# ErikNatanael/knaster

Hardware: AMD Instinct MI355X
Metric: UGen-samples/sec (voices x block_size x UGens / s) (higher is better)
Workload: dtype f32

## Files before the change

knaster_amd/csrc/voice_chain.hpp:

```cpp
#pragma once
#include "voice_stages.hpp"

namespace knh_dev {

template <typename F, bool FMA, int BASE, typename... S> struct Chain;
template <typename F, bool FMA, int BASE>
struct Chain<F, FMA, BASE> {
  static constexpr int kSlots = BASE;
  static constexpr bool kUsesSine = false;
  static constexpr bool kPan = false;
  static constexpr bool kStereo = false;
  static constexpr u64 kParamBits = 0ull, kNopOkBits = 0ull;
  static constexpr bool kBinds = false;
  static constexpr bool kUsesRing = false;
  static constexpr int kRingStages = 0;
  template <int T> __device__ __forceinline__ void tick_tile_sw(const Chain&, u32, u64, F (&)[T], const Ctx&, u32) {}
  __device__ __forceinline__ void pan_gains(F&, F&) const {}
  template <typename W> __device__ __forceinline__ void load(const W*, long) {}
  template <typename W> __device__ __forceinline__ void store(W*, long) const {}
  __device__ __forceinline__ F tick(F x, const Ctx&, u32) { return x; }
  template <int T> __device__ __forceinline__ void tick_tile(F (&)[T], const Ctx&, u32) {}
  struct RunPrep {};
  __device__ __forceinline__ RunPrep prepare_run() const { return RunPrep(); }
  template <int T> __device__ __forceinline__ void tick_tile_run(F (&)[T], const Ctx&, u32, const RunPrep&) {}
#ifdef KNH_DAG_STAMPS
  template <int T> __device__ __forceinline__ void tick_tile_stamped(F (&)[T], const Ctx&, u32, u64*, u64&) {}
#endif
  __device__ __forceinline__ void on_event(u32, u32, u64, u32) {}
  __device__ __forceinline__ bool last_env_stopped(bool dflt) const { return dflt; }
  __device__ __forceinline__ u32 collect_done(u32 acc) const { return acc; }
  __device__ __forceinline__ void reset_marks() {}
  __device__ __forceinline__ void begin_block(u32, const Ctx&) {}
};
template <typename F, bool FMA, int BASE, typename S0, typename... Rest>
struct Chain<F, FMA, BASE, S0, Rest...> {
  typedef Chain<F, FMA, BASE + S0::kSlots, Rest...> RestT;
  static constexpr int kSlots = RestT::kSlots;
  static constexpr bool kUsesSine = S0::kUsesSine || RestT::kUsesSine;
  static constexpr bool kPan = IsPan<S0>::value || RestT::kPan;
  static constexpr bool kStereo = false;
  static constexpr u64 kStageBits = BASE + S0::kSlots <= 64 ? (((u64)1 << S0::kSlots) - 1) << (BASE < 64 ? BASE : 0) : 0ull;
  static constexpr u64 kParamBits = (BASE + S0::kSlots <= 64 ? (u64)S0::kParamMask << (BASE < 64 ? BASE : 0) : 0ull) | RestT::kParamBits;
  static constexpr u64 kNopOkBits = ((S0::kParamMask != 0u || !S0::kHasSeg) && BASE < 64 ? (u64)1 << (BASE < 64 ? BASE : 0) : 0ull) | RestT::kNopOkBits;
  static constexpr bool kBinds = S0::kNeedsBind || RestT::kBinds;
  static constexpr bool kUsesRing = S0::kUsesRing || RestT::kUsesRing;
  static constexpr int kRingStages = (S0::kUsesRing ? 1 : 0) + RestT::kRingStages;
  typename S0::template Regs<F> r;
  u32 mark = 0xFFFFFFFFu;
  RestT rest;
  template <typename W> __device__ __forceinline__ void load(const W* s, long stride) {
    S0::template load<F, W>(r, s + (long)BASE * stride, stride);
    rest.load(s, stride);
  }
  template <typename W> __device__ __forceinline__ void store(W* s, long stride) const {
    S0::template store<F, W>(r, s + (long)BASE * stride, stride);
    rest.store(s, stride);
  }
  __device__ __forceinline__ F tick(F x, const Ctx& c, u32 frame) {
    x = S0::template tick<F, FMA>(r, x, c, frame, mark);
    return rest.tick(x, c, frame);
  }
  template <int T> __device__ __forceinline__ void tick_tile(F (&x)[T], const Ctx& c, u32 frame0) {
    S0::template tick_tile<F, FMA, T>(r, x, c, frame0, mark);
    rest.template tick_tile<T>(x, c, frame0);
  }
  struct RunPrep { bool mine; typename RestT::RunPrep rest; };
  __device__ __forceinline__ RunPrep prepare_run() const {
    RunPrep p;
    if constexpr (S0::kHasRunPrep) p.mine = S0::template prepare_run<F>(r);
    else p.mine = false;
    p.rest = rest.prepare_run();
    return p;
  }
  template <int T> __device__ __forceinline__ void tick_tile_run(F (&x)[T], const Ctx& c, u32 frame0, const RunPrep& p) {
    if constexpr (S0::kHasRunPrep) S0::template tick_tile_prepared<F, FMA, T>(r, x, c, frame0, mark, p.mine);
    else S0::template tick_tile<F, FMA, T>(r, x, c, frame0, mark);
    rest.template tick_tile_run<T>(x, c, frame0, p.rest);
  }
#ifdef KNH_DAG_STAMPS
  template <int T> __device__ __forceinline__ void tick_tile_stamped(F (&x)[T], const Ctx& c, u32 frame0, u64* acc, u64& t_prev) {
    S0::template tick_tile<F, FMA, T>(r, x, c, frame0, mark);
    asm volatile("" : "+v"(x[T - 1]) : : "memory");
    const u64 t = __builtin_amdgcn_s_memtime();
    acc[0] += t - t_prev;
    t_prev = t;
    rest.template tick_tile_stamped<T>(x, c, frame0, acc + 1, t_prev);
  }
#endif
  template <int T> __device__ __forceinline__ void tick_tile_sw(const Chain& cn, u32 sw, u64 touched, F (&x)[T], const Ctx& c, u32 frame0) {
    bool hit = false;
    if constexpr (S0::kParamMask != 0u) hit = __builtin_amdgcn_ballot_w64((touched & kStageBits) != 0ull) != 0;
    if (hit) {
#pragma unroll
      for (int j = 0; j < T; ++j) {
        S0::take_params(r, cn.r, (u32)j == sw);
        x[j] = S0::template tick<F, FMA>(r, x[j], c, frame0 + j, mark);
      }
    } else {
#pragma unroll
      for (int j = 0; j < T; ++j) x[j] = S0::template tick<F, FMA>(r, x[j], c, frame0 + j, mark);
    }
    rest.template tick_tile_sw<T>(cn.rest, sw, touched, x, c, frame0);
  }
  __device__ __forceinline__ u32 collect_done(u32 acc) const {
    if constexpr (S0::kIsEnv) acc = mark != 0xFFFFFFFFu ? mark : acc;
    return rest.collect_done(acc);
  }
  __device__ __forceinline__ void reset_marks() { mark = 0xFFFFFFFFu; rest.reset_marks(); }
  __device__ __forceinline__ void pan_gains(F& l, F& rg) const {
    if constexpr (IsPan<S0>::value) { l = r.l; rg = r.r; }
    else rest.pan_gains(l, rg);
  }
  __device__ __forceinline__ void on_event(u32 op, u32 slot, u64 bits, u32 frame) {
    if (slot >= (u32)BASE && slot < (u32)(BASE + S0::kSlots)) S0::template on_event<F>(r, op, slot - BASE, bits, frame);
    else rest.on_event(op, slot, bits, frame);
  }
  __device__ __forceinline__ bool last_env_stopped(bool dflt) const {
    if constexpr (S0::kIsEnv && !S0::kEnvSource) return rest.last_env_stopped(S0::template is_stopped<F>(r));
    else return rest.last_env_stopped(dflt);
  }
  __device__ __forceinline__ void begin_block(u32 frame_begin, const Ctx& c) {
    if constexpr (S0::kNeedsBind) S0::template bind<F>(r, c);
    if constexpr (S0::kIsEnv && S0::kHasSeg) r.seg = frame_begin;
    rest.begin_block(frame_begin, c);
  }
};

template <int OP>
struct Math2 : StageDefaults {
  static constexpr int kSlots = 0;
  static constexpr u32 kMutableMask = 0u;
  static constexpr bool kUsesSine = false;
  static constexpr bool kIsEnv = false;
  static constexpr bool kNeedsBind = false;
  static constexpr bool kHasSeg = false;
  static constexpr bool kBinary = true;
  template <typename F> struct Regs {};
  template <typename F, typename W> static __device__ __forceinline__ void load(Regs<F>&, const W*, long) {}
  template <typename F, typename W> static __device__ __forceinline__ void store(const Regs<F>&, W*, long) {}
  template <typename F> static __device__ __forceinline__ F apply(F a, F b) {
    if (OP == 0) return a * b;
    if (OP == 1) return a + b;
    if (OP == 2) return a - b;
    if (OP == 3) return a / b;
    return dev_pow(a, b);
  }
  template <typename F, bool FMA> static __device__ __forceinline__ F tick(Regs<F>&, F x, const Ctx&, u32, u32&) { return x; }
  template <typename F, bool FMA, int T> static __device__ __forceinline__ void tick_tile(Regs<F>&, F (&)[T], const Ctx&, u32, u32&) {}
  template <typename F> static __device__ __forceinline__ void on_event(Regs<F>&, u32, u32, u64, u32) {}
};
template <typename S, int A, int B, int O> struct At {};
template <typename S, int A, int B, int O, int O2> struct At2 {};
template <int R> struct Slots {};
template <int R, int K> struct Out1 {};
template <int R, int L, int RR> struct Outs {};
template <typename X> struct NodeOf { static constexpr bool dag = false; };
template <typename S, int A, int B, int O> struct NodeOf<At<S, A, B, O>> { typedef S stage; static constexpr int a = A, b = B, o = O, o2 = -1; static constexpr bool dag = true; };
template <typename S, int A, int B, int O, int O2> struct NodeOf<At2<S, A, B, O, O2>> { typedef S stage; static constexpr int a = A, b = B, o = O, o2 = O2; static constexpr bool dag = true; };
template <int R> struct NodeOf<Slots<R>> { static constexpr bool dag = true; };
template <int R, int K> struct NodeOf<Out1<R, K>> { static constexpr bool dag = true; };
template <int R, int L, int RR> struct NodeOf<Outs<R, L, RR>> { static constexpr bool dag = true; };

template <typename F, bool FMA, int BASE, int R, int LAST, typename... Ns> struct DagChain;
template <typename F, int BASE, int R>
struct DagEnd {
  static constexpr int kSlots = BASE;
  static constexpr bool kUsesSine = false;
  static constexpr bool kPan = false;
  static constexpr bool kUsesRing = false;
  static constexpr int kRingStages = 0;
  __device__ __forceinline__ void pan_gains(F&, F&) const {}
  template <typename W> __device__ __forceinline__ void load(const W*, long) {}
  template <typename W> __device__ __forceinline__ void store(W*, long) const {}
  template <int T> __device__ __forceinline__ void run_tile(F (&)[R][T], const Ctx&, u32) {}
  __device__ __forceinline__ void run_one(F (&)[R], const Ctx&, u32) {}
  __device__ __forceinline__ void on_event(u32, u32, u64, u32) {}
  __device__ __forceinline__ bool last_env_stopped(bool dflt) const { return dflt; }
// ... 1046 lines not shown
```

knaster_amd/csrc/voice_pipe.hpp:

```cpp
#pragma once
#include "voice_chain.hpp"

namespace knh_dev {

template <typename... S> struct Group {};
template <int K, typename... S> struct Fan {};

template <typename G> struct GroupInfo;
template <typename... S> struct GroupInfo<Group<S...>> {
  static constexpr int slots = (0 + ... + S::kSlots);
  static constexpr bool uses_sine = (false || ... || S::kUsesSine);
  static constexpr bool uses_ring = (false || ... || S::kUsesRing);
  static constexpr bool has_env = (false || ... || S::kIsEnv);
  static constexpr bool has_silencer = (false || ... || (S::kIsEnv && !S::kEnvSource));
  static constexpr bool pan = (false || ... || IsPan<S>::value);
  static constexpr int fan_for(int) { return 1; }
};
template <int K, typename... S> struct GroupInfo<Fan<K, S...>> {
  static constexpr int slots = (0 + ... + S::kSlots);
  static constexpr bool uses_sine = (false || ... || S::kUsesSine);
  static constexpr bool uses_ring = false;
  static constexpr bool has_env = false;
  static constexpr bool has_silencer = false;
  static constexpr bool pan = false;
// ... 135 lines not shown
    if (ev_i < ev_end) { nxt = fetch(ev_ranged ? 2u * ev_i : ev_i); note_next(); }
    else { nxt.frame = 0xFFFFFFFFu; next_frame = 0xFFFFFFFFu; }
  };
  u32 base = 0;
  auto apply_events_upto = [&](u32 n_abs) {
    while (__builtin_expect(next_frame <= n_abs, 0)) {
      const u32 op = nxt.slot_op >> 24, slot = nxt.slot_op & 0xFFFFFFu;
      if (slot >= SLOT_LO && slot < SLOT_HI) {
        chain.on_event(op, slot, nxt.bits, nxt.frame - base);
        if (live && (op & 0x7Fu) == EV_SET) a.state[(long)slot * a.stride + voice] = (W)nxt.bits;
      }
      ++ev_i;
      take_next();
    }
  };
  u32 done_frame = 0xFFFFFFFFu;
  for (;;) {
  if (resident) {
    const ResCall call = res_wait(a.res, res_expect, sh.res_slot, wave_all, lane);
    if (call.leave) break;
    res_expect = (res_expect + 1u) & (u32)RES_EPOCH_MASK;
    fbeg = call.frame_begin;
    fend = call.frame_end;
    evs = call.has_events ? a.res.ev_start[call.list] : nullptr;
    ev_g = (glb_ev_t)a.res.events[call.list];
    chain.reset_marks();
    const ResStaged st = res_stage_events(a.res, call, sh.ev_stage, sh.ev_cap, v0, nv, (u32)(wave_all * 64 + lane), sh.n_threads);
    ev_staged = st.count != 0u;
    ev_lds_first = st.first;
    ev_ranged = call.has_events && call.n_ranges != 0u;
    if (ev_ranged) { evs = nullptr; ev_i = 0; ev_end = call.n_ranges; }
  } else if (sh.launch_ranges != 0u) {
    ev_ranged = true;
    ev_i = 0; ev_end = sh.launch_ranges;
  }
  if (!ev_ranged) {
    ev_i = 0; ev_end = 0;
    if (evs) {
      if (resident) { ev_i = *reinterpret_cast<const volatile u32*>(evs + voice); ev_end = *reinterpret_cast<const volatile u32*>(evs + voice + 1); }
      else { ev_i = evs[voice]; ev_end = evs[voice + 1]; }
    }
  }
  nxt.frame = 0xFFFFFFFFu; next_frame = 0xFFFFFFFFu;
  take_next();
  base = 0;

  const u32 n_frames = fend - fbeg;
  const int tpb = (int)((n_frames + T - 1) / T);
  const int n_tiles = tpb * (int)a.n_blocks;
  const int n_steps = n_tiles + NG - (MODE == PIPE_FOLD ? 1 : 0);
  const u32 n_waves_total = (a.n_voices + 63u) / 64u;
  const int full = n_frames >= fo + (u32)TW ? (int)((n_frames - fo - (u32)TW) / (u32)T) + 1 : 0;
  int in_t = Map::in_tile(I, 0), out_t = Map::out_tile(I, 0);
#ifdef KNH_DAG_STAMPS
  u64 busy = 0, busy_in = 0, busy_out = 0, busy_tick = 0, busy_fold = 0;
#endif
  for (int s = 0; s < I; ++s) pipe_barrier();
  for (int blk = 0, ti = 0; blk < (tpb > 0 ? (int)a.n_blocks : 0); ++blk) {
    ctx.input_block = reinterpret_cast<const F*>(a.input) + (long)blk * a.in_channels * a.block_size;
    chain.begin_block(fbeg, ctx);
    for (ti = 0;;) {
      typedef typename EdgeLayout<F, T>::Vec Vec;
      constexpr int VW = EdgeLayout<F, T>::VW;
#ifdef KNH_DAG_STAMPS
      const u64 t0 = __builtin_amdgcn_s_memtime();
#endif
      const u32 n_tile = fbeg + (u32)ti * T;
      const u32 n = n_tile + fo;
      apply_events_upto(base + n);
      const bool ev_inside = next_frame < base + n + TW;
      bool step_open = true;
      if (__builtin_expect(ti < full && !__builtin_amdgcn_ballot_w64(ev_inside), 1)) {
        const typename ChainT::RunPrep prep = chain.prepare_run();
        u32 nq = n;
        for (;;) {
#ifdef KNH_DAG_STAMPS
          const u64 q0 = __builtin_amdgcn_s_memtime();
#endif
          F x[TW];
          if (I > 0) {
            const Vec* in = reinterpret_cast<const Vec*>(sh.edge + (long)in_t * EdgeLayout<F, T>::tile + (long)lane * EdgeLayout<F, T>::stride + fo);
#pragma unroll
            for (int j = 0; j < TW / VW; ++j) {
              const Vec v = in[j];
#pragma unroll
              for (int k = 0; k < VW; ++k) x[j * VW + k] = v[k];
            }
          } else {
#pragma unroll
            for (int j = 0; j < TW; ++j) x[j] = (F)0;
          }
#if defined(KNH_DAG_STAMPS) || defined(KNH_TILE_FENCES)
          asm volatile("s_waitcnt lgkmcnt(0)" ::: "memory");
#endif
#ifdef KNH_DAG_STAMPS
          const u64 q1 = __builtin_amdgcn_s_memtime();
          busy_in += q1 - q0;
#endif
          chain.template tick_tile_run<TW>(x, ctx, nq, prep);
#ifdef KNH_DAG_STAMPS
          asm volatile("" ::: "memory");
          const u64 q2 = __builtin_amdgcn_s_memtime();
          busy_tick += q2 - q1;
#endif
          F* const out_tile = sh.edge + (long)out_t * EdgeLayout<F, T>::tile;
          F* const out_row = out_tile + (long)lane * EdgeLayout<F, T>::stride + fo;
          Vec* out = reinterpret_cast<Vec*>(out_row);
#pragma unroll
          for (int j = 0; j < TW / VW; ++j) {
            Vec v;
#pragma unroll
            for (int k = 0; k < VW; ++k) v[k] = x[j * VW + k];
            out[j] = v;
          }
          if constexpr (GroupInfo<G>::pan) {
            F gl = (F)0, gr = (F)0;
            chain.pan_gains(gl, gr);
            out_row[T] = gl;
            out_row[T + 1] = gr;
          }
#ifdef KNH_DAG_STAMPS
          asm volatile("s_waitcnt lgkmcnt(0)" ::: "memory");
          const u64 qf = __builtin_amdgcn_s_memtime();
#endif
          if constexpr (FOLDS) pipe_fold_tile<F, FMA, T, GroupInfo<G>::pan>(out_tile, a, lane, wave_global, n_waves_total, blk, nq, (u32)T, v0, nv);
#ifdef KNH_DAG_STAMPS
          asm volatile("s_waitcnt lgkmcnt(0)" ::: "memory");
          const u64 qe = __builtin_amdgcn_s_memtime();
          busy_fold += qe - qf;
#endif
          in_t = Map::next_in(I, in_t);
          out_t = Map::next_out(I, out_t);
          nq += (u32)T;
          ++ti;
#if defined(KNH_DAG_STAMPS) || defined(KNH_TILE_FENCES)
          asm volatile("s_waitcnt lgkmcnt(0)" ::: "memory");
#endif
#ifdef KNH_DAG_STAMPS
          const u64 q3 = __builtin_amdgcn_s_memtime();
          busy_out += q3 - qe;
          busy += q3 - q0;
#endif
          if (ti >= full) break;
          pipe_barrier();
          if (__builtin_amdgcn_ballot_w64(next_frame < base + nq + TW)) { step_open = false; break; }
        }
      } else {
        const u32 m_tile = fend - n_tile < (u32)T ? fend - n_tile : (u32)T;
        const u32 m = m_tile > fo ? (m_tile - fo < (u32)TW ? m_tile - fo : (u32)TW) : 0u;
        F* const out_tile = sh.edge + (long)out_t * EdgeLayout<F, T>::tile;
        F* const out_row = out_tile + (long)lane * EdgeLayout<F, T>::stride + fo;
        const F* const in_row = sh.edge + (long)in_t * EdgeLayout<F, T>::tile + (long)lane * EdgeLayout<F, T>::stride + fo;
#ifdef KNH_AB_NO_SW
        if (false && [&]() -> bool {
#else
        if (m == (u32)TW && ChainT::kParamBits != 0ull && !ChainT::kBinds && [&]() -> bool {
#endif
          ChainT cn = chain;
          const u32 sv_i = ev_i;
          const Event sv_nxt = nxt;
          const u32 sv_next_frame = next_frame;
          const u32 tile_end = base + n + (u32)TW;
          u32 sw = (u32)TW;
          u64 touched = 0ull;
          bool bad = false;
          while (next_frame < tile_end) {
            const u32 op = nxt.slot_op >> 24, slot = nxt.slot_op & 0xFFFFFFu, code = op & 0x7Fu;
            if (slot >= SLOT_LO && slot < SLOT_HI) {
              const u32 rel = nxt.frame - (base + n);
              if (sw == (u32)TW) sw = rel;
              bad = bad || sw != rel || slot >= 64u ||
                    !((code == EV_SET && ((ChainT::kParamBits >> (slot & 63u)) & 1ull)) || (code == EV_NOP && ((ChainT::kNopOkBits >> (slot & 63u)) & 1ull)));
              if (!bad) {
                cn.on_event(op, slot, nxt.bits, nxt.frame - base);
                touched |= 1ull << (slot & 63u);
                if (live && code == EV_SET) a.state[(long)slot * a.stride + voice] = (W)nxt.bits;
              }
            }
            ++ev_i;
            take_next();
          }
          if (__builtin_amdgcn_ballot_w64(bad) != 0) {
            ev_i = sv_i;
            nxt = sv_nxt;
            next_frame = sv_next_frame;
            return false;
          }
          for (u32 j0 = 0; j0 < (u32)TW; j0 += 8u) {
            F sub[8];
            if (I > 0) {
#pragma unroll
              for (int q = 0; q < 8 / VW; ++q) {
                const Vec v = reinterpret_cast<const Vec*>(in_row + j0)[q];
#pragma unroll
                for (int k = 0; k < VW; ++k) sub[q * VW + k] = v[k];
              }
            } else {
#pragma unroll
// ... 348 lines not shown
```

knaster_amd/csrc/voice_stages.hpp:

```cpp
#pragma once

extern "C" __device__ float __ocml_sin_f32(float);
extern "C" __device__ double __ocml_sin_f64(double);
extern "C" __device__ float __ocml_cos_f32(float);
extern "C" __device__ double __ocml_cos_f64(double);
extern "C" __device__ float __ocml_pow_f32(float, float);
extern "C" __device__ double __ocml_pow_f64(double, double);
extern "C" __device__ float __ocml_tan_f32(float);
extern "C" __device__ double __ocml_tan_f64(double);
extern "C" __device__ float __ocml_exp_f32(float);
extern "C" __device__ double __ocml_exp_f64(double);
extern "C" __device__ float __ocml_sqrt_f32(float);
extern "C" __device__ double __ocml_sqrt_f64(double);

namespace knh_dev {

typedef unsigned int u32;
typedef unsigned long long u64;

template <typename F> struct WordOf;
template <> struct WordOf<float> { typedef u32 type; };
template <> struct WordOf<double> { typedef u64 type; };

template <typename F> __device__ __forceinline__ F word_to_f(typename WordOf<F>::type w);
template <> __device__ __forceinline__ float word_to_f<float>(u32 w) { return __builtin_bit_cast(float, w); }
template <> __device__ __forceinline__ double word_to_f<double>(u64 w) { return __builtin_bit_cast(double, w); }
__device__ __forceinline__ u32 f_to_word(float f) { return __builtin_bit_cast(u32, f); }
__device__ __forceinline__ u64 f_to_word(double f) { return __builtin_bit_cast(u64, f); }

template <bool FMA> __device__ __forceinline__ float mad(float a, float b, float c) {
  if constexpr (FMA) return __builtin_fmaf(a, b, c);
  else return a * b + c;
}
template <bool FMA> __device__ __forceinline__ double mad(double a, double b, double c) {
  if constexpr (FMA) return __builtin_fma(a, b, c);
  else return a * b + c;
}

__device__ __forceinline__ u32 sat_u32(double v) {
  u32 r;
  asm("v_cvt_u32_f64 %0, %1" : "=v"(r) : "v"(v));
  return r;
}

struct StageDefaults {
  static constexpr u32 kParamMask = 0u;
  template <typename R> static __device__ __forceinline__ void take_params(R&, const R&, bool) {}
  static constexpr bool kBinary = false;
  static constexpr int kArParam = -1;
  static constexpr bool kUsesRing = false;
  static constexpr bool kHasRunPrep = false;
  static constexpr bool kEnvSource = false;
};
template <typename S, int P> struct ArP : S {
  static constexpr int kArParam = P;
};

enum { EV_SET = 0, EV_ENV_ASR_RELEASE = 1, EV_NOP = 2, EV_SEGENV_STOP = 3, EV_ALLPASS_DELAY = 4, EV_SPLIT = 0x80  };

struct Event {
  u32 frame;
  u32 slot_op;
  u64 bits;
};

struct Ctx {
  const float* sine;
  double f2pi;
  const double* seg_table;
  u32 seg_max;
  void* delay_ring;
  u32 delay_stride;
  const void* buffer;
  const void* wavetables;
  const void* input_block;
  u32 in_stride;
  u32 sample_rate;
  __attribute__((address_space(3))) char* ring_tile;
  u32 ring_sink_row;
};


template <bool AR_FREQ>
struct SinWtT : StageDefaults {
  static constexpr int kSlots = 3;
  static constexpr u32 kMutableMask = AR_FREQ ? 0b101u : 0b001u;
  static constexpr bool kUsesSine = true;
  static constexpr bool kIsEnv = false;
  static constexpr bool kNeedsBind = false;
  static constexpr bool kHasSeg = false;
  template <typename F> struct Regs { u32 phase, off, inc; };
  static constexpr u32 kParamMask = AR_FREQ ? 0b010u : 0b110u;
  template <typename R> static __device__ __forceinline__ void take_params(R& r, const R& n, bool c) {
    r.off = c ? n.off : r.off;
    if (!AR_FREQ) r.inc = c ? n.inc : r.inc;
  }
  template <typename F, typename W>
  static __device__ __forceinline__ void load(Regs<F>& r, const W* s, long stride) {
    r.phase = (u32)s[0]; r.off = (u32)s[stride]; r.inc = (u32)s[2 * stride];
  }
  template <typename F, typename W>
  static __device__ __forceinline__ void store(const Regs<F>& r, W* s, long stride) {
    s[0] = (W)r.phase;
    if (AR_FREQ) s[2 * stride] = (W)r.inc;
  }
  template <typename F, int P>
  static __device__ __forceinline__ void ar_set(Regs<F>& r, F v, const Ctx& c) {
    if (P == 0) r.inc = sat_u32((double)v * c.f2pi);
    else r.off = sat_u32((double)v * 65536.0);
  }
  template <typename F, bool FMA>
  static __device__ __forceinline__ F tick(Regs<F>& r, F x, const Ctx& c, u32, u32&) {
    if (AR_FREQ) {
      r.inc = sat_u32((double)x * c.f2pi);
    }
    float s = c.sine[((r.phase + r.off) >> 16) & 16383u];
    r.phase += r.inc;
    return (F)s;
  }
  template <typename F, bool FMA, int T>
  static __device__ __forceinline__ void tick_tile(Regs<F>& r, F (&x)[T], const Ctx& c, u32 frame0, u32& done_frame) {
    if constexpr (AR_FREQ) {
      u32 q = r.phase + r.off, inc = r.inc;
#pragma unroll
      for (int j = 0; j < T; ++j) {
        inc = sat_u32((double)x[j] * c.f2pi);
        x[j] = (F)c.sine[(q >> 16) & 16383u];
        q += inc;
      }
      r.inc = inc;
      r.phase = q - r.off;
    } else {
      u32 q = r.phase + r.off;
#pragma unroll
      for (int j = 0; j < T; ++j) {
        x[j] = (F)c.sine[(q >> 16) & 16383u];
        q += r.inc;
      }
      r.phase = q - r.off;
    }
  }
  template <typename F>
  static __device__ __forceinline__ void on_event(Regs<F>& r, u32 op, u32 rel, u64 bits, u32 ) {
// ... 863 lines not shown
  }
  template <typename F, typename W>
  static __device__ __forceinline__ void store(const Regs<F>& r, W* s, long) { s[0] = f_to_word(r.phase); }
  template <typename F, bool FMA>
  static __device__ __forceinline__ F tick(Regs<F>& r, F, const Ctx&, u32, u32&) {
    const F p = r.phase + r.off;
    r.phase += r.inc;
    if (r.phase > (F)1) r.phase -= (F)1;
    return p;
  }
  template <typename F, bool FMA, int T>
  static __device__ __forceinline__ void tick_tile(Regs<F>& r, F (&x)[T], const Ctx& c, u32 frame0, u32& done_frame) {
#pragma unroll
    for (int j = 0; j < T; ++j) x[j] = tick<F, FMA>(r, x[j], c, frame0 + j, done_frame);
  }
  template <typename F>
  static __device__ __forceinline__ void on_event(Regs<F>& r, u32 op, u32 rel, u64 bits, u32 ) {
    if ((op & 0x7Fu) != EV_SET) return;
    F v = word_to_f<F>((typename WordOf<F>::type)bits);
    if (rel == 0) r.phase = v;
    else if (rel == 1) r.off = v;
    else r.inc = v;
  }
};
struct SinMap : StageDefaults {
  static constexpr int kSlots = 0;
  static constexpr u32 kMutableMask = 0u;
  static constexpr bool kUsesSine = false;
  static constexpr bool kIsEnv = false;
  static constexpr bool kNeedsBind = false;
  static constexpr bool kHasSeg = false;
  template <typename F> struct Regs {};
  template <typename F, typename W> static __device__ __forceinline__ void load(Regs<F>&, const W*, long) {}
  template <typename F, typename W> static __device__ __forceinline__ void store(const Regs<F>&, W*, long) {}
  template <typename F, bool FMA>
  static __device__ __forceinline__ F tick(Regs<F>&, F p, const Ctx&, u32, u32&) {
    return SinNum::sin_turns(p);
  }
  template <typename F, bool FMA, int T>
  static __device__ __forceinline__ void tick_tile(Regs<F>& r, F (&x)[T], const Ctx& c, u32 frame0, u32& done_frame) {
#pragma unroll
    for (int j = 0; j < T; ++j) x[j] = tick<F, FMA>(r, x[j], c, frame0 + j, done_frame);
  }
  template <typename F> static __device__ __forceinline__ void on_event(Regs<F>&, u32, u32, u64, u32) {}
};

struct Svf : StageDefaults {
  static constexpr int kSlots = 8;
  static constexpr u32 kMutableMask = 0b11u;
  static constexpr bool kUsesSine = false;
  static constexpr bool kIsEnv = false;
  static constexpr bool kNeedsBind = false;
  static constexpr bool kHasSeg = false;
  template <typename F> struct Regs { F ic1, ic2, a1, a2, a3, m1, m2; typename WordOf<F>::type nl; F m0; };
  template <typename R> static __device__ __forceinline__ void note_mix(R& r) {
    r.nl = (f_to_word(r.m0) | f_to_word(r.m1)) | (f_to_word(r.m2) ^ f_to_word((decltype(r.m2))1));
  }
  static constexpr u32 kParamMask = 0b11111100u;
  template <typename R> static __device__ __forceinline__ void take_params(R& r, const R& n, bool c) {
    r.a1 = c ? n.a1 : r.a1; r.a2 = c ? n.a2 : r.a2; r.a3 = c ? n.a3 : r.a3;
    r.m0 = c ? n.m0 : r.m0; r.m1 = c ? n.m1 : r.m1; r.m2 = c ? n.m2 : r.m2;
    r.nl = c ? n.nl : r.nl;
  }
  template <typename F, typename W>
  static __device__ __forceinline__ void load(Regs<F>& r, const W* s, long st) {
    r.ic1 = word_to_f<F>(s[0]); r.ic2 = word_to_f<F>(s[st]); r.a1 = word_to_f<F>(s[2 * st]);
    r.a2 = word_to_f<F>(s[3 * st]); r.a3 = word_to_f<F>(s[4 * st]); r.m0 = word_to_f<F>(s[5 * st]);
    r.m1 = word_to_f<F>(s[6 * st]); r.m2 = word_to_f<F>(s[7 * st]);
    note_mix(r);
  }
  template <typename F, typename W>
  static __device__ __forceinline__ void store(const Regs<F>& r, W* s, long st) {
    s[0] = f_to_word(r.ic1); s[st] = f_to_word(r.ic2);
  }
  template <typename F, bool FMA>
  static __device__ __forceinline__ F tick(Regs<F>& r, F v0, const Ctx&, u32, u32&) {
    const F v3 = v0 - r.ic2;
    if constexpr (FMA) {
      const F v1 = mad<true>(r.a2, v3, r.a1 * r.ic1);
      const F v2 = mad<true>(r.a3, v3, mad<true>(r.a2, r.ic1, r.ic2));
      r.ic1 = mad<true>((F)2, v1, -r.ic1);
      r.ic2 = mad<true>((F)2, v2, -r.ic2);
      return mad<true>(r.m2, v2, mad<true>(r.m1, v1, r.m0 * v0));
    } else {
      const F v1 = r.a1 * r.ic1 + r.a2 * v3;
      const F v2 = r.ic2 + r.a2 * r.ic1 + r.a3 * v3;
      r.ic1 = mad<true>((F)2, v1, -r.ic1);
      r.ic2 = mad<true>((F)2, v2, -r.ic2);
      return r.m0 * v0 + r.m1 * v1 + r.m2 * v2;
    }
  }
#ifdef KNH_SVF_NOP
#define KNH_SVF_WAIT "s_nop 0\n\t"
#else
#define KNH_SVF_WAIT
#endif
  static constexpr int kHighestFixedVgpr = 122;
  template <int T>
  static __device__ __forceinline__ void tick_tile_packed(Regs<float>& r, float (&x)[T]) {
    static_assert(T % 8 == 0, "the filter tile is unrolled in blocks of eight samples");
    static_assert(kHighestFixedVgpr < 128, "the fixed registers stay inside the smallest register budget of any kernel form (128: __launch_bounds__(1024))");
    float ic1 = r.ic1, ic2 = r.ic2;
    const float a1 = r.a1, a2 = r.a2, a2b = r.a2, a3 = r.a3, m0 = r.m0, m1 = r.m1, m2 = r.m2;
#define KNH_SVF_STEP(K)                                                                                            \
      "v_sub_f32 v114, %[x" #K "], v101\n\t"                                 \
      "v_pk_mul_f32 v[102:103], v[116:117], v[100:101] op_sel_hi:[1,0]\n\t"      \
// ... 98 lines not shown
      KNH_STEP(const double p1 = a1 * ic1);
      KNH_STEP(const double p2 = a2 * ic1);
      if (j > 0) { KNH_STEP(o1 = m1 * v1p); }
      KNH_STEP(const double q1 = a2 * v3);
      KNH_STEP(const double q2 = a3 * v3);
      KNH_STEP(const double t = ic2 + p2);
      if (j > 0) { KNH_STEP(o2 = m2 * v2p); }
      KNH_STEP(const double v1 = p1 + q1);
      KNH_STEP(const double v2 = t + q2);
      if (j > 0) { KNH_STEP(s = o0p + o1); }
      KNH_STEP(ic1 = __builtin_fma(2.0, v1, -ic1));
      KNH_STEP(ic2 = __builtin_fma(2.0, v2, -ic2));
      KNH_STEP(const double o0 = m0 * x[j]);
      if (j > 0) { KNH_STEP(x[j - 1] = s + o2); }
      v1p = v1; v2p = v2; o0p = o0;
    }
    x[T - 1] = (o0p + m1 * v1p) + m2 * v2p;
#undef KNH_STEP
    r.ic1 = ic1; r.ic2 = ic2;
  }
  static constexpr bool kHasRunPrep = true;
  template <typename F> static __device__ __forceinline__ bool prepare_run(const Regs<F>& r) { return low_pass(r); }
  template <typename F, bool FMA, int T>
  static __device__ __forceinline__ void tick_tile_prepared(Regs<F>& r, F (&x)[T], const Ctx& c, u32 frame0, u32& done_frame, bool low) {
    if constexpr (sizeof(F) == 4 && !FMA) {
      if (low) tick_tile_low<T>(r, x); else tick_tile_packed<T>(r, x);
    } else if constexpr (sizeof(F) == 8 && !FMA) {
      if (low) tick_tile_low_f64<T>(r, x); else tick_tile_f64<T>(r, x);
    } else {
#pragma unroll
      for (int j = 0; j < T; ++j) x[j] = tick<F, FMA>(r, x[j], c, frame0 + j, done_frame);
    }
  }
  template <typename F, bool FMA, int T>
  static __device__ __forceinline__ void tick_tile(Regs<F>& r, F (&x)[T], const Ctx& c, u32 frame0, u32& done_frame) {
    tick_tile_prepared<F, FMA, T>(r, x, c, frame0, done_frame, low_pass(r));
  }
  template <typename F>
  static __device__ __forceinline__ void on_event(Regs<F>& r, u32 op, u32 rel, u64 bits, u32 ) {
    if ((op & 0x7Fu) != EV_SET) return;
    F v = word_to_f<F>((typename WordOf<F>::type)bits);
    r.ic1 = rel == 0 ? v : r.ic1; r.ic2 = rel == 1 ? v : r.ic2; r.a1 = rel == 2 ? v : r.a1; r.a2 = rel == 3 ? v : r.a2;
    r.a3 = rel == 4 ? v : r.a3; r.m0 = rel == 5 ? v : r.m0; r.m1 = rel == 6 ? v : r.m1; r.m2 = rel >= 7 ? v : r.m2;
    note_mix(r);
  }
};

static __device__ __forceinline__ float dev_pow(float a, float b) { return __ocml_pow_f32(a, b); }
static __device__ __forceinline__ double dev_pow(double a, double b) { return __ocml_pow_f64(a, b); }
struct SvfP : Svf {
  static constexpr int kSlots = 12;
  static constexpr u32 kParamMask = 0u;
  static constexpr bool kHasRunPrep = false;
  template <typename F> struct Regs : Svf::Regs<F> { F cutoff, q, gain; u32 ty; };
  template <typename F, typename W>
  static __device__ __forceinline__ void load(Regs<F>& r, const W* s, long st) {
    Svf::load<F, W>(r, s, st);
    r.cutoff = word_to_f<F>(s[8 * st]); r.q = word_to_f<F>(s[9 * st]); r.gain = word_to_f<F>(s[10 * st]); r.ty = (u32)s[11 * st];
  }
  template <typename F, typename W>
  static __device__ __forceinline__ void store(const Regs<F>& r, W* s, long st) {
    Svf::store<F, W>(r, s, st);
    s[2 * st] = f_to_word(r.a1); s[3 * st] = f_to_word(r.a2); s[4 * st] = f_to_word(r.a3);
    s[5 * st] = f_to_word(r.m0); s[6 * st] = f_to_word(r.m1); s[7 * st] = f_to_word(r.m2);
    s[8 * st] = f_to_word(r.cutoff); s[9 * st] = f_to_word(r.q); s[10 * st] = f_to_word(r.gain);
  }
  static __device__ __forceinline__ float tan_f(float v) { return __ocml_tan_f32(v); }
  static __device__ __forceinline__ double tan_f(double v) { return __ocml_tan_f64(v); }
  static __device__ __forceinline__ float sqrt_f(float v) { return __ocml_sqrt_f32(v); }
  static __device__ __forceinline__ double sqrt_f(double v) { return __ocml_sqrt_f64(v); }
  template <typename F>
  static __device__ __forceinline__ void set_coeffs(Regs<F>& r, const Ctx& c) {
    const F one = (F)1, sr = (F)(float)c.sample_rate;
    F g = tan_f(((F)3.14159265358979323846 * r.cutoff) / sr);
    F k = one / r.q;
    F m0 = (F)0, m1 = (F)0, m2 = (F)0, amp = (F)0;
    if (r.ty >= 6u && r.ty <= 8u) amp = dev_pow((F)10, r.gain / (F)40);
    switch (r.ty) {
      default: m2 = one; break;
      case 2u: m1 = one; break;
      case 1u: m0 = one; m1 = -k; m2 = -one; break;
      case 3u: m0 = one; m1 = -k; break;
      case 4u: m0 = one; m1 = -k; m2 = -(F)2; break;
      case 5u: m0 = one; m1 = -(F)2 * k; break;
      case 6u: g = g / sqrt_f(amp); k = one / (r.q * amp); m0 = one; m1 = k * (amp * amp - one); break;
      case 7u: g = g / sqrt_f(amp); m0 = one; m1 = k * (amp - one); m2 = amp * amp - one; break;
      case 8u: g = g * sqrt_f(amp); m0 = amp * amp; m1 = k * (one - amp) * amp; m2 = one - amp * amp; break;
    }
    r.a1 = one / (one + g * (g + k));
    r.a2 = g * r.a1;
    r.a3 = g * r.a2;
    r.m0 = m0; r.m1 = m1; r.m2 = m2;
  }
  template <typename F, int P>
  static __device__ __forceinline__ void ar_set(Regs<F>& r, F v, const Ctx& c) {
    if (P == 0) r.cutoff = v; else if (P == 1) r.q = v; else r.gain = v;
    set_coeffs<F>(r, c);
  }
  template <typename F, bool FMA>
  static __device__ __forceinline__ F tick(Regs<F>& r, F v0, const Ctx& c, u32 n, u32& d) { return Svf::tick<F, FMA>(r, v0, c, n, d); }
  template <typename F, bool FMA, int T>
  static __device__ __forceinline__ void tick_tile(Regs<F>& r, F (&x)[T], const Ctx& c, u32 frame0, u32& done_frame) {
#pragma unroll
    for (int j = 0; j < T; ++j) x[j] = Svf::tick<F, FMA>(r, x[j], c, frame0 + j, done_frame);
  }
  template <typename F>
// ... 12 lines not shown
  static constexpr bool kUsesSine = false;
  static constexpr bool kIsEnv = false;
  static constexpr bool kNeedsBind = false;
  static constexpr bool kHasSeg = false;
  template <typename F> struct Regs { F y, a0, b1; };
  static constexpr u32 kParamMask = 0b110u;
  template <typename R> static __device__ __forceinline__ void take_params(R& r, const R& n, bool c) {
    r.a0 = c ? n.a0 : r.a0;
    r.b1 = c ? n.b1 : r.b1;
  }
  template <typename F, typename W>
  static __device__ __forceinline__ void load(Regs<F>& r, const W* s, long st) {
    r.y = word_to_f<F>(s[0]); r.a0 = word_to_f<F>(s[st]); r.b1 = word_to_f<F>(s[2 * st]);
  }
  template <typename F, typename W>
  static __device__ __forceinline__ void store(const Regs<F>& r, W* s, long) { s[0] = f_to_word(r.y); }
  static __device__ __forceinline__ float exp_f(float v) { return __ocml_exp_f32(v); }
  static __device__ __forceinline__ double exp_f(double v) { return __ocml_exp_f64(v); }
  template <typename F, int P>
  static __device__ __forceinline__ void ar_set(Regs<F>& r, F v, const Ctx& c) {
    const F f = v / (F)c.sample_rate;
    r.b1 = exp_f((F)-2.0 * (F)3.14159265358979323846 * f);
    r.a0 = (F)1.0 - r.b1;
  }
  template <typename F, bool FMA>
  static __device__ __forceinline__ F tick(Regs<F>& r, F x, const Ctx&, u32, u32&) {
    if constexpr (FMA) r.y = mad<true>(x, r.a0, r.y * r.b1);
    else r.y = x * r.a0 + r.y * r.b1;
    return HIGHPASS ? x - r.y : r.y;
  }
  template <typename F, bool FMA, int T>
  static __device__ __forceinline__ void tick_tile(Regs<F>& r, F (&x)[T], const Ctx& c, u32 frame0, u32& done_frame) {
#pragma unroll
    for (int j = 0; j < T; ++j) x[j] = tick<F, FMA>(r, x[j], c, frame0 + j, done_frame);
  }
  template <typename F>
  static __device__ __forceinline__ void on_event(Regs<F>& r, u32 op, u32 rel, u64 bits, u32 ) {
    if ((op & 0x7Fu) != EV_SET) return;
    F v = word_to_f<F>((typename WordOf<F>::type)bits);
    if (rel == 0) r.y = v; else if (rel == 1) r.a0 = v; else r.b1 = v;
  }
};
typedef OnePoleT<false> OnePoleLp;
typedef OnePoleT<true> OnePoleHp;

template <bool AR>
struct MulEnvT : StageDefaults {
  static constexpr int kSlots = 5;
  static constexpr u32 kMutableMask = 0b10011u;
  static constexpr bool kUsesSine = false;
  static constexpr bool kIsEnv = true;
  static constexpr bool kNeedsBind = false;
  static constexpr bool kHasSeg = true;
  template <typename F> struct Regs { u32 state; F t, ar, rr, scale; u32 seg; };
  static constexpr u32 kParamMask = 0b01100u;
  template <typename R> static __device__ __forceinline__ void take_params(R& r, const R& n, bool c) {
    r.ar = c ? n.ar : r.ar;
    r.rr = c ? n.rr : r.rr;
    r.seg = c ? n.seg : r.seg;
  }
  template <typename F> static __device__ __forceinline__ bool is_stopped(const Regs<F>& r) { return r.state == 0u; }
  template <typename F, typename W>
  static __device__ __forceinline__ void load(Regs<F>& r, const W* s, long st) {
    r.state = (u32)s[0]; r.t = word_to_f<F>(s[st]); r.ar = word_to_f<F>(s[2 * st]);
    r.rr = word_to_f<F>(s[3 * st]); r.scale = word_to_f<F>(s[4 * st]);
    r.seg = 0;
  }
  template <typename F, typename W>
  static __device__ __forceinline__ void store(const Regs<F>& r, W* s, long st) {
    s[0] = (W)r.state; s[st] = f_to_word(r.t); s[4 * st] = f_to_word(r.scale);
  }
  template <typename F, int P>
  static __device__ __forceinline__ void ar_set(Regs<F>& r, F v, const Ctx& c) {
    const F rate = v == (F)0 ? (F)1 : (F)1 / (v * (F)c.sample_rate);
    if (P == 0) r.ar = rate; else r.rr = rate;
  }
  template <typename F>
  static __device__ __forceinline__ F env_next(Regs<F>& r, u32 frame, u32& done_frame) {
    const u32 st = r.state;
    const F t = r.t;
    const F rel_out = (t * (t * t)) * r.scale;
    F env = (F)0;
    if (st == 1u) env = t;
    if (st == 2u) env = (F)1;
    if (st == 3u) env = rel_out;
    if (st == 1u) {
      F nt = t + r.ar;
      r.t = nt;
      if (nt >= (F)1) {
        if (AR) { r.scale = (F)1; r.state = 3u; r.t = (F)1; }
        else r.state = 2u;
      }
    } else if (st == 3u) {
      F nt = t - r.rr;
      r.t = nt;
      if (nt <= (F)0) { r.state = 0u; r.t = (F)0; done_frame = frame - r.seg; }
    }
    return env;
  }
  template <typename F, bool FMA>
  static __device__ __forceinline__ F tick(Regs<F>& r, F x, const Ctx&, u32 frame, u32& done_frame) {
    return x * env_next<F>(r, frame, done_frame);
  }
  template <bool MUL, typename F> static __device__ __forceinline__ F put(F x, F e) { return MUL ? x * e : e; }
  template <typename F, int T, bool MUL>
  static __device__ __forceinline__ void release_tile_clamped(F (&x)[T], F& t_io, F step, F scale, F (&t_block)[T / 8]) {
// ... 674 lines not shown
          const Vec v = src[j];
#pragma unroll
          for (int k = 0; k < VW; ++k) y[j * VW + k] = v[k];
        }
        F wr[T];
#pragma unroll
        for (int j = 0; j < T; ++j) {
          const F d = allpass<F>(r, y[j]);
          wr[j] = FB ? d * r.fb + x[j] : x[j];
          x[j] = FB ? d - r.fb * wr[j] : d;
        }
        Vec* dst = reinterpret_cast<Vec*>(r.ring + r.wp);
#pragma unroll
        for (int j = 0; j < T / VW; ++j) {
          Vec v;
#pragma unroll
          for (int k = 0; k < VW; ++k) v[k] = wr[j * VW + k];
          dst[j] = v;
        }
        r.rp = r.rp + (u32)T == r.len ? 0u : r.rp + (u32)T;
        r.wp = r.wp + (u32)T == r.len ? 0u : r.wp + (u32)T;
      }
      return;
    }
#pragma unroll
    for (int j = 0; j < T; ++j) x[j] = tick<F, FMA>(r, x[j], c, frame0 + j, done_frame);
  }
  template <typename F>
  static __device__ __forceinline__ void on_event(Regs<F>& r, u32 op, u32 rel, u64 bits, u32) {
    op &= 0x7Fu;
    if (op == EV_ALLPASS_DELAY) {
      const u32 nf = (u32)bits;
      r.rp = r.wp >= nf ? r.wp - nf : r.len - nf + r.wp;
      return;
    }
    if (op != EV_SET) return;
    if (rel == 4) r.coeff = word_to_f<F>((typename WordOf<F>::type)bits);
    else if (rel == 7) r.fb = word_to_f<F>((typename WordOf<F>::type)bits);
    else if (rel == 0) r.wp = (u32)bits;
    else if (rel == 1) r.rp = (u32)bits;
  }
};
typedef AllpassDelayT<false> AllpassDelay;
typedef AllpassDelayT<true> AllpassFbDelay;

template <int OP>
struct ValT : StageDefaults {
  static constexpr int kSlots = 1;
  static constexpr u32 kMutableMask = 0u;
  static constexpr bool kUsesSine = false;
  static constexpr bool kIsEnv = false;
  static constexpr bool kNeedsBind = false;
  static constexpr bool kHasSeg = false;
  template <typename F> struct Regs { F v; };
  static constexpr u32 kParamMask = 0b1u;
  template <typename R> static __device__ __forceinline__ void take_params(R& r, const R& n, bool c) { r.v = c ? n.v : r.v; }
  template <typename F, typename W>
  static __device__ __forceinline__ void load(Regs<F>& r, const W* s, long) { r.v = word_to_f<F>(s[0]); }
  template <typename F, typename W>
  static __device__ __forceinline__ void store(const Regs<F>&, W*, long) {}
  template <typename F, int P>
  static __device__ __forceinline__ void ar_set(Regs<F>& r, F v, const Ctx&) { r.v = v; }
  template <typename F, bool FMA>
  static __device__ __forceinline__ F tick(Regs<F>& r, F x, const Ctx&, u32, u32&) {
    if (OP == 0) return x * r.v;
    if (OP == 1) return x + r.v;
    if (OP == 2) return x - r.v;
    if (OP == 3) return x / r.v;
    if (OP == 4) return r.v - x;
    if (OP == 5) return r.v / x;
    return dev_pow(x, r.v);
  }
  template <typename F, bool FMA, int T>
  static __device__ __forceinline__ void tick_tile(Regs<F>& r, F (&x)[T], const Ctx& c, u32 frame0, u32& done_frame) {
    if constexpr (sizeof(F) == 4 && OP <= 2 && T % 2 == 0) {
      typedef float f2 __attribute__((ext_vector_type(2)));
      const f2 v = {r.v, r.v};
#pragma unroll
      for (int j = 0; j < T; j += 2) {
        f2 p = {x[j], x[j + 1]};
        p = OP == 0 ? p * v : (OP == 1 ? p + v : p - v);
        x[j] = p.x; x[j + 1] = p.y;
      }
    } else {
#pragma unroll
      for (int j = 0; j < T; ++j) x[j] = tick<F, FMA>(r, x[j], c, frame0 + j, done_frame);
    }
  }
  template <typename F>
  static __device__ __forceinline__ void on_event(Regs<F>& r, u32 op, u32, u64 bits, u32 ) {
    if ((op & 0x7Fu) == EV_SET) r.v = word_to_f<F>((typename WordOf<F>::type)bits);
  }
};
typedef ValT<0> MulVal;
typedef ValT<1> AddVal;
typedef ValT<2> SubVal;
typedef ValT<3> DivVal;
typedef ValT<4> VSubVal;
typedef ValT<5> VDivVal;
typedef ValT<6> PowVal;

struct PowiVal : StageDefaults {
  static constexpr int kSlots = 1;
  static constexpr u32 kMutableMask = 0u;
  static constexpr bool kUsesSine = false;
  static constexpr bool kIsEnv = false;
  static constexpr bool kNeedsBind = false;
  static constexpr bool kHasSeg = false;
  template <typename F> struct Regs { int n; };
  static constexpr u32 kParamMask = 0b1u;
  template <typename R> static __device__ __forceinline__ void take_params(R& r, const R& n, bool c) { r.n = c ? n.n : r.n; }
  template <typename F, typename W>
  static __device__ __forceinline__ void load(Regs<F>& r, const W* s, long) { r.n = (int)(u32)s[0]; }
  template <typename F, typename W>
  static __device__ __forceinline__ void store(const Regs<F>&, W*, long) {}
  template <typename F, bool FMA>
  static __device__ __forceinline__ F tick(Regs<F>& r, F x, const Ctx&, u32, u32&) {
    u32 p = r.n < 0 ? 0u - (u32)r.n : (u32)r.n;
    F a = x, m = (F)1;
    for (;;) {
      if (p & 1u) m *= a;
      p >>= 1;
      if (p == 0u) break;
      a *= a;
    }
    return r.n < 0 ? (F)1 / m : m;
  }
  template <typename F, bool FMA, int T>
  static __device__ __forceinline__ void tick_tile(Regs<F>& r, F (&x)[T], const Ctx& c, u32 frame0, u32& done_frame) {
#pragma unroll
    for (int j = 0; j < T; ++j) x[j] = tick<F, FMA>(r, x[j], c, frame0 + j, done_frame);
  }
  template <typename F>
  static __device__ __forceinline__ void on_event(Regs<F>& r, u32 op, u32, u64 bits, u32) {
    if ((op & 0x7Fu) == EV_SET) r.n = (int)(u32)bits;
  }
};

struct Pan2 : StageDefaults {
  static constexpr int kSlots = 2;
  static constexpr u32 kMutableMask = 0u;
  static constexpr bool kUsesSine = false;
  static constexpr bool kIsEnv = false;
  static constexpr bool kNeedsBind = false;
  static constexpr bool kHasSeg = false;
  template <typename F> struct Regs { F l, r; };
  template <typename F, typename W>
  static __device__ __forceinline__ void load(Regs<F>& r, const W* s, long st) { r.l = word_to_f<F>(s[0]); r.r = word_to_f<F>(s[st]); }
  template <typename F, typename W>
  static __device__ __forceinline__ void store(const Regs<F>&, W*, long) {}
  template <typename F, bool FMA>
  static __device__ __forceinline__ F tick(Regs<F>&, F x, const Ctx&, u32, u32&) { return x; }
  template <typename F, bool FMA, int T>
  static __device__ __forceinline__ void tick_tile(Regs<F>&, F (&)[T], const Ctx&, u32, u32&) {}
  template <typename F>
  static __device__ __forceinline__ void on_event(Regs<F>& r, u32 op, u32 rel, u64 bits, u32) {
    if ((op & 0x7Fu) != EV_SET) return;
    const F v = word_to_f<F>((typename WordOf<F>::type)bits);
    if (rel == 0) r.l = v; else r.r = v;
  }
};
template <typename S> struct IsPan { static constexpr bool value = false; };
template <> struct IsPan<Pan2> { static constexpr bool value = true; };

}
```

Measured before the change: 3299 billion.

## Run fast tile path across block boundaries when chain has no per-block work

Adds a per-stage kHasBlockWork flag and a chain-level kBlockWork, plus a check that env segments are already at the block start. When no stage needs per-block work, the fast run loop continues into following blocks without leaving the inner loop. This skips the outer step machinery and the begin_block handling at each block edge. It also moves the event-due check ahead of the barrier and drops the barrier on early exit, which changes synchronisation order and adds control-flow complexity.

```diff
diff --git a/knaster_amd/csrc/voice_chain.hpp b/knaster_amd/csrc/voice_chain.hpp
--- a/knaster_amd/csrc/voice_chain.hpp
+++ b/knaster_amd/csrc/voice_chain.hpp
@@ -12,6 +12,7 @@
   static constexpr bool kStereo = false;
   static constexpr u64 kParamBits = 0ull, kNopOkBits = 0ull;
   static constexpr bool kBinds = false;
+  static constexpr bool kBlockWork = false;
   static constexpr bool kUsesRing = false;
   static constexpr int kRingStages = 0;
   template <int T> __device__ __forceinline__ void tick_tile_sw(const Chain&, u32, u64, F (&)[T], const Ctx&, u32) {}
@@ -31,6 +32,7 @@
   __device__ __forceinline__ u32 collect_done(u32 acc) const { return acc; }
   __device__ __forceinline__ void reset_marks() {}
   __device__ __forceinline__ void begin_block(u32, const Ctx&) {}
+  __device__ __forceinline__ bool block_begun(u32) const { return true; }
 };
 template <typename F, bool FMA, int BASE, typename S0, typename... Rest>
 struct Chain<F, FMA, BASE, S0, Rest...> {
@@ -43,6 +45,7 @@
   static constexpr u64 kParamBits = (BASE + S0::kSlots <= 64 ? (u64)S0::kParamMask << (BASE < 64 ? BASE : 0) : 0ull) | RestT::kParamBits;
   static constexpr u64 kNopOkBits = ((S0::kParamMask != 0u || !S0::kHasSeg) && BASE < 64 ? (u64)1 << (BASE < 64 ? BASE : 0) : 0ull) | RestT::kNopOkBits;
   static constexpr bool kBinds = S0::kNeedsBind || RestT::kBinds;
+  static constexpr bool kBlockWork = S0::kHasBlockWork || S0::kNeedsBind || RestT::kBlockWork;
   static constexpr bool kUsesRing = S0::kUsesRing || RestT::kUsesRing;
   static constexpr int kRingStages = (S0::kUsesRing ? 1 : 0) + RestT::kRingStages;
   typename S0::template Regs<F> r;
@@ -123,6 +126,11 @@
     if constexpr (S0::kNeedsBind) S0::template bind<F>(r, c);
     if constexpr (S0::kIsEnv && S0::kHasSeg) r.seg = frame_begin;
     rest.begin_block(frame_begin, c);
+  }
+  __device__ __forceinline__ bool block_begun(u32 frame_begin) const {
+    bool ok = rest.block_begun(frame_begin);
+    if constexpr (S0::kIsEnv && S0::kHasSeg) ok = ok && r.seg == frame_begin;
+    return ok;
   }
 };
 
diff --git a/knaster_amd/csrc/voice_pipe.hpp b/knaster_amd/csrc/voice_pipe.hpp
--- a/knaster_amd/csrc/voice_pipe.hpp
+++ b/knaster_amd/csrc/voice_pipe.hpp
@@ -211,6 +211,9 @@
   const u32 n_waves_total = (a.n_voices + 63u) / 64u;
   const int full = n_frames >= fo + (u32)TW ? (int)((n_frames - fo - (u32)TW) / (u32)T) + 1 : 0;
   int in_t = Map::in_tile(I, 0), out_t = Map::out_tile(I, 0);
+  constexpr bool CROSS = !ChainT::kBlockWork;
+  const bool cross_ok = CROSS && !resident && n_frames != 0u && n_frames % (u32)T == 0u;
+  const u32 wrap_gap = a.block_size - n_frames;
 #ifdef KNH_DAG_STAMPS
   u64 busy = 0, busy_in = 0, busy_out = 0, busy_tick = 0, busy_fold = 0;
 #endif
@@ -231,78 +234,101 @@
       bool step_open = true;
       if (__builtin_expect(ti < full && !__builtin_amdgcn_ballot_w64(ev_inside), 1)) {
         const typename ChainT::RunPrep prep = chain.prepare_run();
+        int cross_left = 0;
+        if constexpr (CROSS) {
+          if (cross_ok && !__builtin_amdgcn_ballot_w64(!chain.block_begun(fbeg))) cross_left = (int)a.n_blocks - 1 - blk;
+        }
         u32 nq = n;
+        u32 due = base + n + (u32)TW;
         for (;;) {
-#ifdef KNH_DAG_STAMPS
-          const u64 q0 = __builtin_amdgcn_s_memtime();
-#endif
-          F x[TW];
-          if (I > 0) {
-            const Vec* in = reinterpret_cast<const Vec*>(sh.edge + (long)in_t * EdgeLayout<F, T>::tile + (long)lane * EdgeLayout<F, T>::stride + fo);
+          for (;;) {
+#ifdef KNH_DAG_STAMPS
+            const u64 q0 = __builtin_amdgcn_s_memtime();
+#endif
+            F x[TW];
+            if (I > 0) {
+              const Vec* in = reinterpret_cast<const Vec*>(sh.edge + (long)in_t * EdgeLayout<F, T>::tile + (long)lane * EdgeLayout<F, T>::stride + fo);
+#pragma unroll
+              for (int j = 0; j < TW / VW; ++j) {
+                const Vec v = in[j];
+#pragma unroll
+                for (int k = 0; k < VW; ++k) x[j * VW + k] = v[k];
+              }
+            } else {
+#pragma unroll
+              for (int j = 0; j < TW; ++j) x[j] = (F)0;
+            }
+#if defined(KNH_DAG_STAMPS) || defined(KNH_TILE_FENCES)
+            asm volatile("s_waitcnt lgkmcnt(0)" ::: "memory");
+#endif
+#ifdef KNH_DAG_STAMPS
+            const u64 q1 = __builtin_amdgcn_s_memtime();
+            busy_in += q1 - q0;
+#endif
+            chain.template tick_tile_run<TW>(x, ctx, nq, prep);
+#ifdef KNH_DAG_STAMPS
+            asm volatile("" ::: "memory");
+            const u64 q2 = __builtin_amdgcn_s_memtime();
+            busy_tick += q2 - q1;
+#endif
+            F* const out_tile = sh.edge + (long)out_t * EdgeLayout<F, T>::tile;
+            F* const out_row = out_tile + (long)lane * EdgeLayout<F, T>::stride + fo;
+            Vec* out = reinterpret_cast<Vec*>(out_row);
 #pragma unroll
             for (int j = 0; j < TW / VW; ++j) {
-              const Vec v = in[j];
-#pragma unroll
-              for (int k = 0; k < VW; ++k) x[j * VW + k] = v[k];
-            }
-          } else {
-#pragma unroll
-            for (int j = 0; j < TW; ++j) x[j] = (F)0;
+              Vec v;
+#pragma unroll
+              for (int k = 0; k < VW; ++k) v[k] = x[j * VW + k];
+              out[j] = v;
+            }
+            if constexpr (GroupInfo<G>::pan) {
+              F gl = (F)0, gr = (F)0;
+              chain.pan_gains(gl, gr);
+              out_row[T] = gl;
+              out_row[T + 1] = gr;
+            }
+#ifdef KNH_DAG_STAMPS
+            asm volatile("s_waitcnt lgkmcnt(0)" ::: "memory");
+            const u64 qf = __builtin_amdgcn_s_memtime();
+#endif
+            if constexpr (FOLDS) pipe_fold_tile<F, FMA, T, GroupInfo<G>::pan>(out_tile, a, lane, wave_global, n_waves_total, blk, nq, (u32)T, v0, nv);
+#ifdef KNH_DAG_STAMPS
+            asm volatile("s_waitcnt lgkmcnt(0)" ::: "memory");
+            const u64 qe = __builtin_amdgcn_s_memtime();
+            busy_fold += qe - qf;
+#endif
+            in_t = Map::next_in(I, in_t);
+            out_t = Map::next_out(I, out_t);
+            nq += (u32)T;
+            due += (u32)T;
+            ++ti;
+#if defined(KNH_DAG_STAMPS) || defined(KNH_TILE_FENCES)
+            asm volatile("s_waitcnt lgkmcnt(0)" ::: "memory");
+#endif
+#ifdef KNH_DAG_STAMPS
+            const u64 q3 = __builtin_amdgcn_s_memtime();
+            busy_out += q3 - qe;
+            busy += q3 - q0;
+#endif
+            if constexpr (CROSS) {
+              if (ti >= full) break;
+              if (__builtin_amdgcn_ballot_w64(next_frame < due)) break;
+              pipe_barrier();
+            } else {
+              if (ti >= full) break;
+              pipe_barrier();
+              if (__builtin_amdgcn_ballot_w64(next_frame < base + nq + TW)) { step_open = false; break; }
+            }
           }
-#if defined(KNH_DAG_STAMPS) || defined(KNH_TILE_FENCES)
-          asm volatile("s_waitcnt lgkmcnt(0)" ::: "memory");
-#endif
-#ifdef KNH_DAG_STAMPS
-          const u64 q1 = __builtin_amdgcn_s_memtime();
-          busy_in += q1 - q0;
-#endif
-          chain.template tick_tile_run<TW>(x, ctx, nq, prep);
-#ifdef KNH_DAG_STAMPS
-          asm volatile("" ::: "memory");
-          const u64 q2 = __builtin_amdgcn_s_memtime();
-          busy_tick += q2 - q1;
-#endif
-          F* const out_tile = sh.edge + (long)out_t * EdgeLayout<F, T>::tile;
-          F* const out_row = out_tile + (long)lane * EdgeLayout<F, T>::stride + fo;
-          Vec* out = reinterpret_cast<Vec*>(out_row);
-#pragma unroll
-          for (int j = 0; j < TW / VW; ++j) {
-            Vec v;
-#pragma unroll
-            for (int k = 0; k < VW; ++k) v[k] = x[j * VW + k];
-            out[j] = v;
-          }
-          if constexpr (GroupInfo<G>::pan) {
-            F gl = (F)0, gr = (F)0;
-            chain.pan_gains(gl, gr);
-            out_row[T] = gl;
-            out_row[T + 1] = gr;
-          }
-#ifdef KNH_DAG_STAMPS
-          asm volatile("s_waitcnt lgkmcnt(0)" ::: "memory");
-          const u64 qf = __builtin_amdgcn_s_memtime();
-#endif
-          if constexpr (FOLDS) pipe_fold_tile<F, FMA, T, GroupInfo<G>::pan>(out_tile, a, lane, wave_global, n_waves_total, blk, nq, (u32)T, v0, nv);
-#ifdef KNH_DAG_STAMPS
-          asm volatile("s_waitcnt lgkmcnt(0)" ::: "memory");
-          const u64 qe = __builtin_amdgcn_s_memtime();
-          busy_fold += qe - qf;
-#endif
-          in_t = Map::next_in(I, in_t);
-          out_t = Map::next_out(I, out_t);
-          nq += (u32)T;
-          ++ti;
-#if defined(KNH_DAG_STAMPS) || defined(KNH_TILE_FENCES)
-          asm volatile("s_waitcnt lgkmcnt(0)" ::: "memory");
-#endif
-#ifdef KNH_DAG_STAMPS
-          const u64 q3 = __builtin_amdgcn_s_memtime();
-          busy_out += q3 - qe;
-          busy += q3 - q0;
-#endif
-          if (ti >= full) break;
+          if (!CROSS || ti < full || cross_left == 0) break;
+          --cross_left;
+          due += wrap_gap;
+          if (__builtin_amdgcn_ballot_w64(next_frame < due)) break;
+          nq = fbeg + fo;
+          ti = 0;
+          ++blk;
+          base += a.block_size;
           pipe_barrier();
-          if (__builtin_amdgcn_ballot_w64(next_frame < base + nq + TW)) { step_open = false; break; }
         }
       } else {
         const u32 m_tile = fend - n_tile < (u32)T ? fend - n_tile : (u32)T;
diff --git a/knaster_amd/csrc/voice_stages.hpp b/knaster_amd/csrc/voice_stages.hpp
--- a/knaster_amd/csrc/voice_stages.hpp
+++ b/knaster_amd/csrc/voice_stages.hpp
@@ -50,6 +50,7 @@
   static constexpr int kArParam = -1;
   static constexpr bool kUsesRing = false;
   static constexpr bool kHasRunPrep = false;
+  static constexpr bool kHasBlockWork = true;
   static constexpr bool kEnvSource = false;
 };
 template <typename S, int P> struct ArP : S {
@@ -89,6 +90,7 @@
   static constexpr bool kIsEnv = false;
   static constexpr bool kNeedsBind = false;
   static constexpr bool kHasSeg = false;
+  static constexpr bool kHasBlockWork = false;
   template <typename F> struct Regs { u32 phase, off, inc; };
   static constexpr u32 kParamMask = AR_FREQ ? 0b010u : 0b110u;
   template <typename R> static __device__ __forceinline__ void take_params(R& r, const R& n, bool c) {
@@ -1058,6 +1060,7 @@
   static constexpr bool kIsEnv = false;
   static constexpr bool kNeedsBind = false;
   static constexpr bool kHasSeg = false;
+  static constexpr bool kHasBlockWork = false;
   template <typename F> struct Regs { F ic1, ic2, a1, a2, a3, m1, m2; typename WordOf<F>::type nl; F m0; };
   template <typename R> static __device__ __forceinline__ void note_mix(R& r) {
     r.nl = (f_to_word(r.m0) | f_to_word(r.m1)) | (f_to_word(r.m2) ^ f_to_word((decltype(r.m2))1));
@@ -1262,6 +1265,7 @@
   static constexpr int kSlots = 12;
   static constexpr u32 kParamMask = 0u;
   static constexpr bool kHasRunPrep = false;
+  static constexpr bool kHasBlockWork = true;
   template <typename F> struct Regs : Svf::Regs<F> { F cutoff, q, gain; u32 ty; };
   template <typename F, typename W>
   static __device__ __forceinline__ void load(Regs<F>& r, const W* s, long st) {
@@ -1380,6 +1384,7 @@
   static constexpr bool kIsEnv = true;
   static constexpr bool kNeedsBind = false;
   static constexpr bool kHasSeg = true;
+  static constexpr bool kHasBlockWork = false;
   template <typename F> struct Regs { u32 state; F t, ar, rr, scale; u32 seg; };
   static constexpr u32 kParamMask = 0b01100u;
   template <typename R> static __device__ __forceinline__ void take_params(R& r, const R& n, bool c) {
@@ -2160,6 +2165,7 @@
   static constexpr bool kIsEnv = false;
   static constexpr bool kNeedsBind = false;
   static constexpr bool kHasSeg = false;
+  static constexpr bool kHasBlockWork = false;
   template <typename F> struct Regs { F v; };
   static constexpr u32 kParamMask = 0b1u;
   template <typename R> static __device__ __forceinline__ void take_params(R& r, const R& n, bool c) { r.v = c ? n.v : r.v; }
@@ -2252,6 +2258,7 @@
   static constexpr bool kIsEnv = false;
   static constexpr bool kNeedsBind = false;
   static constexpr bool kHasSeg = false;
+  static constexpr bool kHasBlockWork = false;
   template <typename F> struct Regs { F l, r; };
   template <typename F, typename W>
   static __device__ __forceinline__ void load(Regs<F>& r, const W* s, long st) { r.l = word_to_f<F>(s[0]); r.r = word_to_f<F>(s[st]); }
```

Measured after the change: 3416 billion, median of 6. +3.5%, better.
